# albertgassol1/vf-nerf

Measured on AMD Instinct MI355X. Metric: rays/sec (4096-ray chunk, 128 samples/ray) + PSNR vs ref, higher is better.
Workload: dtype f16x3+f32acc

## Files before the change

vf_nerf_amd/csrc/vfn_mlp16.hip:

```cpp
#include <string.h>
#include <utility>
#include "vfn_common.h"
#include "vfn_plan.h"

typedef _Float16 half8 __attribute__((ext_vector_type(8)));
typedef _Float16 half2v __attribute__((ext_vector_type(2)));
typedef float float2v __attribute__((ext_vector_type(2)));
typedef float f32x16 __attribute__((ext_vector_type(16)));
typedef float f32x4v __attribute__((ext_vector_type(4)));

constexpr float VFN16_WSCALE = 64.0f;
constexpr float VFN16_INV_WSCALE = 0.015625f;
constexpr float VFN16_XSCALE = 64.0f;
constexpr int VFN16_SAVE_AUX = 2;
constexpr int VFN16_HANDOVER_NUM = 8;
constexpr int VFN16_DMA_STEPS = 16;
constexpr int VFN16_EPI_PER_MFMA = 6;
constexpr int VFN16_EPI_PER_MFMA2 = 9;
#define VFN16_MAX_CHUNK_KB 39
#define VFN16_STATS_WORDS 64

struct Plan16 {
    int32_t n_hidden;
    int32_t feat_layer;
// ... 180 lines not shown
        }
    }
    {
        Pack16Entry& e = a.e[a.n_entries++];
        rc = fill(e, L - 1);
        if (rc != VFN_OK) return rc;
        e.off_kb = p.head_off_kb; e.n_chunks = 1; e.act16 = 16; e.aux16 = 0;
        e.row_off = 0; e.n_rows = 3; e.act_col_off = 0; e.act_valid = VFN_HIDDEN;
    }
    a.total_words = p.total_kb * 256u;
    a.out = (uint32_t*)packed16;
    a.stats = a.out + a.total_words;
    if (hipMemsetAsync(a.stats, 0, VFN16_STATS_WORDS * 4, (hipStream_t)stream) != hipSuccess) {
        vfn_set_error("vfn_pack16_weights: hipMemsetAsync failed");
        return VFN_ERR_LAUNCH;
    }
    hipLaunchKernelGGL(vfn_pack16_kernel, dim3(a.total_words / 256 + VFN16_STAT_WGS * a.n_entries), dim3(256), 0, (hipStream_t)stream, a);
    return vfn_check_launch("vfn_pack16_weights");
}

namespace {

enum : int { EPI_RELU = 0, EPI_TANH = 1, EPI_HEAD_TANH = 2, EPI_HEAD_SIGMOID = 3 };
enum : int { M16_FEAT = 1, M16_RENDER = 2, M16_TRAIN = 4, M16_BLKOUT = 8, M16_BLKIN = 16, M16_C2 = 32, M16_P1 = 64, M16_SF16 = 128,
             M16_VF_VEC = 0, M16_FUSED = M16_FEAT | M16_RENDER, M16_VF_BLK = M16_FEAT | M16_BLKOUT, M16_RN_BLK = M16_RENDER | M16_BLKIN,
             M16_VF_VEC_TRAIN = M16_TRAIN, M16_VF_FULL_TRAIN = M16_FEAT | M16_TRAIN, M16_FUSED_TRAIN = M16_FUSED | M16_TRAIN };

constexpr int VFN16_FDEPTH = 2;
#define VFN16_SLOT (VFN16_MAX_CHUNK_KB * 64)
#define VFN16_WAVES 4
#define VFN16_PTS 128

typedef __attribute__((address_space(3))) void lds_void;

constexpr int VF_ACT[9] = {0, 16, 16, 16, 14, 16, 16, 16, 16};
constexpr int VF_AUX[9] = {3, 0, 0, 0, 3, 0, 0, 0, 0};
constexpr int VF_TILES[9] = {8, 8, 8, 7, 8, 8, 8, 8, 8};
constexpr int RN_ACT[4] = {16, 16, 16, 16};
constexpr int RN_AUX[4] = {3, 0, 0, 0};
constexpr int RN_TILES[4] = {8, 8, 8, 8};
constexpr int HEAD_KB = 2 * 16 + 1;
constexpr int chunk_kb(int act, int aux) { return 2 * (act + aux) + 1; }
constexpr int vf_off_kb(int h) { int o = 0; for (int i = 0; i < h; ++i) o += VF_TILES[i] * chunk_kb(VF_ACT[i], VF_AUX[i]); return o; }
constexpr int rn_off_kb(int h) { int o = 0; for (int i = 0; i < h; ++i) o += RN_TILES[i] * chunk_kb(RN_ACT[i], RN_AUX[i]); return o; }

struct ChunkD { int net, off_kb, kb, aux; };
constexpr ChunkD chunk_of(int mode, int c) {
    if (!(mode & M16_BLKIN)) {
        const int vf_layers = (mode & M16_FEAT) ? 9 : 8;
        for (int h = 0; h < vf_layers; ++h) {
            if (c < VF_TILES[h]) return {0, vf_off_kb(h) + c * chunk_kb(VF_ACT[h], VF_AUX[h]), chunk_kb(VF_ACT[h], VF_AUX[h]), VF_AUX[h]};
            c -= VF_TILES[h];
        }
        if (c == 0) return {0, vf_off_kb(9), HEAD_KB, 0};
        c -= 1;
    }
    if (mode & M16_RENDER) {
        for (int h = 0; h < 4; ++h) {
            if (c < RN_TILES[h]) return {1, rn_off_kb(h) + c * chunk_kb(RN_ACT[h], RN_AUX[h]), chunk_kb(RN_ACT[h], RN_AUX[h]), RN_AUX[h]};
            c -= RN_TILES[h];
        }
        if (c == 0) return {1, rn_off_kb(4), HEAD_KB, 0};
    }
    return {0, 0, 0, 0};
}

constexpr int rn_first_chunk(int mode) { return (mode & M16_BLKIN) ? 0 : 72; }
constexpr bool chunk_two(int mode, int c) { return (mode & M16_C2) && !(mode & M16_BLKIN) && c >= 63 && c != 71; }
constexpr bool mode_one(int mode) { return (mode & M16_P1) != 0; }
constexpr int VFN16_P1_RING = 5;
#define VFN16_P1_SLOT_KB 20
constexpr int ring_of(int mode) { return mode_one(mode) ? VFN16_P1_RING : 3; }
constexpr int slot_u4(int mode) { return mode_one(mode) ? VFN16_P1_SLOT_KB * 64 : VFN16_MAX_CHUNK_KB * 64; }
constexpr int slot_base(int mode, int c) { return (c % ring_of(mode)) * slot_u4(mode); }
static_assert(VFN16_P1_RING * VFN16_P1_SLOT_KB <= 3 * VFN16_MAX_CHUNK_KB, "the single-product ring must fit into the split modes' ring");
constexpr int stores_of(int mode, int c) { return (c == 0 || ((mode & M16_RENDER) && c == rn_first_chunk(mode))) ? 0 : 4; }
constexpr int young_ops(int mode, int c) {
    const int ring = ring_of(mode);
    int n = 0;
    for (int k = (c - ring + 2 > 0 ? c - ring + 2 : 0); k < c; ++k) n += stores_of(mode, k);
    for (int j = 2; j <= ring - 2; ++j)
        if (c + j >= ring - 1 && chunk_of(mode, c + j).kb > 0) n += (((chunk_of(mode, c + j).kb - 1) / 2 + 1) / VFN16_WAVES);
    return n;
}

struct Mlp16Args {
    const uint4* vf_w;
    const uint4* rn_w;
    const float* points;
    const float* ray_dirs;
    float* out_vec;
    float* out_colors;
    long long n_points;
    int dirs_div;
    int vf_multires, rn_multires;
    uint32_t vf_bytes, rn_bytes;
    float* saved;
    float* save_aux_vf;
    float* save_aux_rn;
    uint32_t* save_masks;
    int save_f16;
    uint4* blk_out;
    const uint4* blk_in;
    const float* vec_in;
    const int* src;
    const int* out_index;
    long long ws_first, ws_points;
    uint32_t* status;
    const int* n_dev;
    unsigned long long* clock;
    long long clock_slots;
};

#define VFN16_CLAMP 60000.0f
constexpr int VFN16_CLAMP_BITS = 0x476a6000;
static_assert(__builtin_bit_cast(int, VFN16_CLAMP) == VFN16_CLAMP_BITS, "VFN16_CLAMP_BITS is VFN16_CLAMP as an integer");

struct X16 { half8 hi[16]; half8 lo[16]; };
struct A16 { half8 hi[3]; half8 lo[3]; };

struct Pipe16 {
    uint4* lds;
    __amdgpu_buffer_rsrc_t vf_w;
    __amdgpu_buffer_rsrc_t rn_w;
    float* saved;
    long long slot_floats;
    uint32_t slot_bytes;
    uint32_t save_voff;
    uint32_t save_voff16;
    uint32_t feat_voff;
    uint32_t st_tile, st_q;
    int save16;
    uint32_t* masks;
    uint32_t mask_bytes;
    uint32_t mask_voff;
    uint4* blk_out;
    uint32_t blk_bytes, blk_voff;
};

struct Carry16 {
    f32x16 pend;
    f32x16 bias;
    half8 fh0, fl0;
    uint32_t lm[4];
    unsigned long long sat;
};

template <int N, typename F, int... I>
__device__ __forceinline__ void static_for_impl(F&& f, std::integer_sequence<int, I...>) { (f(std::integral_constant<int, I>{}), ...); }
template <int N, typename F>
__device__ __forceinline__ void static_for(F&& f) { static_for_impl<N>(f, std::make_integer_sequence<int, N>{}); }

__device__ __forceinline__ void split2(float a, float b, _Float16& h0, _Float16& h1, _Float16& l0, _Float16& l1) {
    const float2v v = {a, b};
    const half2v hi = __builtin_convertvector(v, half2v);
    h0 = hi[0]; h1 = hi[1];
    const uint32_t hp = __builtin_bit_cast(uint32_t, hi);
    float r0, r1;
    asm("v_fma_mix_f32 %0, %1, -1.0, %2 op_sel_hi:[1,0,0]" : "=v"(r0) : "v"(hp), "v"(a));
    asm("v_fma_mix_f32 %0, %1, -1.0, %2 op_sel:[1,0,0] op_sel_hi:[1,0,0]" : "=v"(r1) : "v"(hp), "v"(b));
    const float2v r = {r0, r1};
    const half2v lo = __builtin_convertvector(r, half2v);
    l0 = lo[0]; l1 = lo[1];
}

__device__ __forceinline__ float tanh_exp(float v) { return 1.0f - 2.0f / (1.0f + expf(2.0f * v)); }
// ... 221 lines not shown
                else asm volatile("s_waitcnt vmcnt(0)" ::: "memory");
                __builtin_amdgcn_s_barrier();
            }
            if (st >= H && st < H + DST && ddma.kb > 0) {
#pragma unroll
                for (int i = (st - H) * PM / DST; i < (st - H + 1) * PM / DST; ++i) {
                    if (VFN16_WAVES * i + VFN16_WAVES <= DPIECES) dma_piece<ddma.net, ddma.off_kb, slot_base(MODE, C + RING - 1)>(p, piece_blk(wave + VFN16_WAVES * i), lane, P1 ? wave + VFN16_WAVES * i : -1);
                    else if (VFN16_WAVES * i < DPIECES) {
                        const int idx = min(wave + VFN16_WAVES * i, DPIECES - 1);
                        dma_piece<ddma.net, ddma.off_kb, slot_base(MODE, C + RING - 1)>(p, piece_blk(idx), lane, P1 ? idx : -1);
                    }
                }
            }
            if (TRAIN && MPARTS > 0 && st >= H && st < H + MPARTS && (ch > 0 || PEPI >= 0)) {
                static_for<MPARTS>([&](auto ip) {
                    constexpr int part = decltype(ip)::value;
                    if (st - H == part) {
                        if (ch > 0) collect_mask_part<(ch > 0 ? ch - 1 : 0), EPI, part, (MPARTS > 0 ? MPARTS : 1)>(cy, mbits);
                        else collect_mask_part<PKB / 2, (PEPI >= 0 ? PEPI : 0), part, (MPARTS > 0 ? MPARTS : 1)>(cy, mbits);
                    }
                });
            }
            if (TRAIN && st >= DEND && st < DEND + SSTEPS && (ch > 0 || PEPI >= 0)) {
                if (st == DEND) {
                    if constexpr (MPARTS > 0) {
                        if (ch == 0) store_mask<(PSLOT >= 0 ? PSLOT : 0)>(p, cy);
                    } else {
                        if (ch > 0) collect_mask<(ch > 0 ? ch - 1 : 0), EPI>(cy);
                        else { collect_mask<PKB / 2, (PEPI >= 0 ? PEPI : 0)>(cy); store_mask<(PSLOT >= 0 ? PSLOT : 0)>(p, cy); }
                    }
                }
#pragma unroll
                for (int q = (st - DEND) * 4 / SSTEPS; q < (st - DEND + 1) * 4 / SSTEPS; ++q) {
                    if (ch > 0) save_group<(SLOT >= 0 ? SLOT : 0), (ch > 0 ? ch - 1 : 0), (MODE & M16_SF16) != 0>(p, cy.pend, q);
                    else save_group<(PSLOT >= 0 ? PSLOT : 0), PKB / 2, (MODE & M16_SF16) != 0>(p, cy.pend, q);
                }
            }
            if (st == H && ((BLK && ch > 0) || (PBLK && ch == 0))) {
                if (ch > 0) store_blocks<(ch > 0 ? ch - 1 : 0)>(p, xout);
                else store_blocks<PKB / 2>(p, xpend);
            }
            if (st == NKB - 1 && dnext.kb > 0) prefetch_chunk<MODE, (dnext.kb > 0 ? C + 1 : C)>(cy, p, lane);
            __builtin_amdgcn_sched_barrier(0);
        }
        if (EPI == EPI_RELU || EPI == EPI_TANH) {
            cy.pend = acc;
        } else {
#pragma unroll
            for (int c = 0; c < 3; ++c) {
                const float v = acc[c] * VFN16_INV_WSCALE;
                head[c] = (EPI == EPI_HEAD_TANH) ? tanh_exp(v) : 1.0f / (1.0f + expf(-v));
            }
        }
    });
}

constexpr int ENC_RT = -1;
constexpr int VFN16_VF_MULTIRES = 6, VFN16_RN_MULTIRES = 4;
constexpr int enc_multires(int fixed, int run_time) { return fixed >= 0 ? fixed : run_time; }

__device__ __forceinline__ void lane_half_pair(float v, float& low, float& high) {
    const unsigned u = __builtin_bit_cast(unsigned, v);
    const auto r = __builtin_amdgcn_permlane32_swap(u, u, false, false);
    low = __builtin_bit_cast(float, (unsigned)r[0]); high = __builtin_bit_cast(float, (unsigned)r[1]);
}

__device__ __forceinline__ float enc_value(const float (&x)[3], const float (&sn)[18], const float (&cs)[18], int multires, int k) {
    if (k < 3) return x[k];
    const int idx = k - 3, oct = idx / 6, rem = idx - 6 * oct;
    if (oct >= multires) return 0.f;
    return rem < 3 ? sn[3 * oct + rem] : cs[3 * oct + rem - 3];
}

template <int NDEF, int NRAW, typename F>
__device__ __forceinline__ void build_aux(A16& aux, int g, F col, float& ain) {
    static_for<3>([&](auto is) {
        constexpr int s = decltype(is)::value;
        half8 hi, lo;
        static_for<4>([&](auto ij) {
            constexpr int j = 2 * decltype(ij)::value;
            if constexpr (16 * s + j >= NDEF) {
                hi[j] = (_Float16)0.f; hi[j + 1] = (_Float16)0.f; lo[j] = (_Float16)0.f; lo[j + 1] = (_Float16)0.f;
            } else {
                float v0, v1;
                if (g == 0) { v0 = col(16 * s + j); v1 = col(16 * s + j + 1); }
                else { v0 = col(16 * s + 8 + j); v1 = col(16 * s + 8 + j + 1); }
                v0 *= VFN16_XSCALE; v1 *= VFN16_XSCALE;
                v0 = fminf(fmaxf(v0, -VFN16_CLAMP), VFN16_CLAMP); v1 = fminf(fmaxf(v1, -VFN16_CLAMP), VFN16_CLAMP);
                if constexpr (16 * s + j < NRAW) ain = fmaxf(ain, fmaxf(fabsf(v0), fabsf(v1)));
                _Float16 h0, h1, l0, l1;
                split2(v0, v1, h0, h1, l0, l1);
                hi[j] = h0; hi[j + 1] = h1; lo[j] = l0; lo[j + 1] = l1;
            }
        });
        aux.hi[s] = hi; aux.lo[s] = lo;
    });
}

template <typename F>
__device__ __forceinline__ void save_aux(float* dst, long long m, int g, F col) {
#pragma unroll
    for (int s = 0; s < 3; ++s)
#pragma unroll
        for (int h = 0; h < 2; ++h) {
            const int c0 = 16 * s + 8 * g + 4 * h;
            if (c0 + 4 <= VFN_AUX_K) {
                f32x4v v;
                if (g == 0) { v = f32x4v{col(16 * s + 4 * h), col(16 * s + 4 * h + 1), col(16 * s + 4 * h + 2), col(16 * s + 4 * h + 3)}; }
                else { v = f32x4v{col(16 * s + 8 + 4 * h), col(16 * s + 8 + 4 * h + 1), col(16 * s + 8 + 4 * h + 2), col(16 * s + 8 + 4 * h + 3)}; }
                *reinterpret_cast<f32x4v*>(dst + m * VFN_AUX_K + c0) = v;
            }
        }
}

__device__ __forceinline__ void load_aux(A16& ax, const float* park) {
    const half8* pk = reinterpret_cast<const half8*>(park + 8);
#pragma unroll
    for (int q = 0; q < 3; ++q) { ax.hi[q] = pk[2 * q]; ax.lo[q] = pk[2 * q + 1]; }
}

template <int MR>
__device__ __forceinline__ void encode_sincos(const float (&x)[3], int multires_rt, int g, float (&sn)[18], float (&cs)[18]) {
    const int multires = enc_multires(MR, multires_rt);
#pragma unroll
    for (int j = 0; j < 3; ++j)
#pragma unroll
        for (int c = 0; c < 3; ++c) {
            if (MR >= 0 && 2 * j >= MR) {
                sn[6 * j + c] = 0.f; cs[6 * j + c] = 0.f; sn[6 * j + 3 + c] = 0.f; cs[6 * j + 3 + c] = 0.f;
                continue;
            }
            float s = 0.f, k = 0.f;
            if (2 * j < multires) {
                sincosf(x[c] * (g ? (float)(2 << (2 * j)) : (float)(1 << (2 * j))), &s, &k);
                if (g && 2 * j + 1 >= multires) { s = 0.f; k = 0.f; }
            }
            lane_half_pair(s, sn[6 * j + c], sn[6 * j + 3 + c]);
            lane_half_pair(k, cs[6 * j + c], cs[6 * j + 3 + c]);
        }
}

template <int MODE, int RNM>
__device__ __forceinline__ void render_aux(const Mlp16Args& a, A16& aux, const float (&xr)[3], const float (&dr)[3], const float (&nrm)[3],
                                           long long m, bool in, int g, float& ain) {
    const int rn_multires = enc_multires(RNM, a.rn_multires);
    float sn[18], cs[18];
    encode_sincos<RNM>(dr, rn_multires, g, sn, cs);
    const int ncol = 6 + 6 * rn_multires;
    auto rn_col = [&](int k) -> float {
        if (k < 3) return xr[k];
        if (k >= ncol) return k < ncol + 3 ? nrm[k - ncol] : 0.f;
        return enc_value(dr, sn, cs, rn_multires, k - 3);
    };
    build_aux<(RNM >= 0 ? 9 + 6 * RNM : 48), 6>(aux, g, rn_col, ain);
    if ((MODE & M16_TRAIN) && in) save_aux(a.save_aux_rn, m, g, rn_col);
}

template <int MODE>
__device__ __forceinline__ void render_tail(const Mlp16Args& a, const Pipe16& p, Carry16& cy, X16& xa, X16& xb, const A16& aux,
                                            const float (&nrm)[3], long long m, bool in, int wave, int lane) {
    constexpr int R = EPI_RELU, NONE = -1;
    constexpr int C0 = rn_first_chunk(MODE);
    float rgb[3] = {0.f, 0.f, 0.f};
    layer16<MODE, C0 + 0, 16, 3, 8, R, NONE, 0, 9, -1>(xb, aux, xa, xb, cy, rgb, p, wave, lane);
    layer16<MODE, C0 + 8, 16, 0, 8, R, R, 14, 10, 9>(xa, aux, xb, xa, cy, rgb, p, wave, lane);
    layer16<MODE, C0 + 16, 16, 0, 8, R, R, 14, 11, 10>(xb, aux, xa, xb, cy, rgb, p, wave, lane);
    layer16<MODE, C0 + 24, 16, 0, 8, R, R, 14, 12, 11>(xa, aux, xb, xa, cy, rgb, p, wave, lane);
    layer16<MODE, C0 + 32, 16, 0, 1, EPI_HEAD_SIGMOID, R, 14, -1, 12>(xb, aux, xa, xb, cy, rgb, p, wave, lane);
    const long long mo = m;
    if (in && (threadIdx.x & 32) == 0) {
        a.out_vec[mo * 3 + 0] = nrm[0]; a.out_vec[mo * 3 + 1] = nrm[1]; a.out_vec[mo * 3 + 2] = nrm[2];
        a.out_colors[mo * 3 + 0] = rgb[0]; a.out_colors[mo * 3 + 1] = rgb[1]; a.out_colors[mo * 3 + 2] = rgb[2];
    }
}

__device__ __forceinline__ void report_range(const Mlp16Args& a, unsigned long long sat, float ain) {
    if (a.status) {
        const unsigned bits = (sat != 0ull ? 1u : 0u) | (ain >= VFN16_CLAMP ? 2u : 0u);
        if (bits) atomicOr(a.status, bits);
    }
}

template <int MODE, int VFM, int RNM>
__device__ __forceinline__ void mlp16_body(const Mlp16Args& a) {
    __shared__ __attribute__((aligned(16))) uint4 s_ring[3 * VFN16_SLOT + 256 * 8];
    float* s_park = reinterpret_cast<float*>(s_ring + 3 * VFN16_SLOT) + threadIdx.x * 32;
    const int tid = threadIdx.x;
    const int lane = tid & 63;
    const int wave = __builtin_amdgcn_readfirstlane(tid >> 6);
    const int g = lane >> 5;
    unsigned long long ck_t0 = 0ull, ck_r0 = 0ull;
    if constexpr ((MODE & M16_RENDER) != 0 && (MODE & M16_BLKIN) == 0 && (MODE & M16_TRAIN) == 0) {
        if (a.clock) { ck_t0 = __builtin_amdgcn_s_memtime(); ck_r0 = __builtin_amdgcn_s_memrealtime(); }
    }
    const long long m = (long long)blockIdx.x * VFN16_PTS + wave * 32 + (lane & 31);
    long long n_live = a.n_points;
    if (a.n_dev) {
        const long long nd = (long long)*a.n_dev;
        n_live = nd < n_live ? nd : n_live;
        if ((long long)blockIdx.x * VFN16_PTS >= n_live) return;
    }
    const bool in = m < n_live;

    if constexpr ((MODE & M16_BLKIN) != 0) {
        const int dpos = in ? a.src[m] : -1;
        const bool live = dpos >= 0;
        float xr[3] = {0.f, 0.f, 0.f}, dr[3] = {0.f, 0.f, 0.f}, nrm[3] = {0.f, 0.f, 0.f};
        if (live) {
            const long long di = dpos / a.dirs_div;
#pragma unroll
            for (int c = 0; c < 3; ++c) { xr[c] = a.points[(long long)dpos * 3 + c]; dr[c] = a.ray_dirs[di * 3 + c]; nrm[c] = a.vec_in[m * 3 + c]; }
        }
        Pipe16 p;
        p.lds = s_ring;
        p.vf_w = __builtin_amdgcn_make_buffer_rsrc(const_cast<uint4*>(a.rn_w), 0, (int)a.rn_bytes, 0x00020000);
        p.rn_w = p.vf_w;
        p.saved = nullptr; p.slot_floats = 0; p.slot_bytes = 0; p.save_voff = 0; p.blk_out = nullptr; p.blk_bytes = 0; p.blk_voff = 0;
        p.masks = nullptr; p.mask_bytes = 0; p.mask_voff = 0; p.save16 = 0; p.save_voff16 = 0; p.feat_voff = 0; p.st_tile = 0; p.st_q = 0;
        dma_chunk<MODE, 0>(p, wave, lane);
        dma_chunk<MODE, 1>(p, wave, lane);
        X16 xa, xb;
        A16 aux;
        float ain_blk = 0.f;
        {
            typedef unsigned int u32x4 __attribute__((ext_vector_type(4)));
            const __amdgpu_buffer_rsrc_t rs_blk = __builtin_amdgcn_make_buffer_rsrc(
                const_cast<uint4*>(a.blk_in), 0, (int)(((a.n_points + 31) & ~31ll) * 1024), 0x00020000);
            const unsigned goff = in ? (unsigned)((m >> 5) * 32768 + lane * 16) : 0xfffffff0u;
            u32x4 q[32];
#pragma unroll
            for (int i = 0; i < 32; ++i) q[i] = __builtin_amdgcn_raw_buffer_load_b128(rs_blk, goff, i * 1024, 0);
            render_aux<MODE, RNM>(a, aux, xr, dr, nrm, -1, false, g, ain_blk);
#pragma unroll
            for (int t = 0; t < 8; ++t) {
                half8 h0 = __builtin_bit_cast(half8, q[4 * t + 0]), l0 = __builtin_bit_cast(half8, q[4 * t + 1]);
                half8 h1 = __builtin_bit_cast(half8, q[4 * t + 2]), l1 = __builtin_bit_cast(half8, q[4 * t + 3]);
                asm volatile("" : "+a"(h0)); asm volatile("" : "+a"(l0)); asm volatile("" : "+a"(h1)); asm volatile("" : "+a"(l1));
                xb.hi[2 * t] = h0; xb.lo[2 * t] = l0; xb.hi[2 * t + 1] = h1; xb.lo[2 * t + 1] = l1;
            }
        }
        asm volatile("s_waitcnt vmcnt(0)" ::: "memory");
        __builtin_amdgcn_s_barrier();
        Carry16 cy;
#pragma unroll
        for (int q = 0; q < 16; ++q) cy.pend[q] = 0.f;
        cy.lm[0] = 0; cy.lm[1] = 0; cy.lm[2] = 0; cy.lm[3] = 0; cy.sat = 0ull;
        prefetch_chunk<MODE, 0>(cy, p, lane);
        render_tail<MODE>(a, p, cy, xa, xb, aux, nrm, live ? (long long)dpos : -1, live, wave, lane);
        report_range(a, cy.sat, ain_blk);
    } else {
    float x[3] = {0.f, 0.f, 0.f};
    if (in) { x[0] = a.points[m * 3 + 0]; x[1] = a.points[m * 3 + 1]; x[2] = a.points[m * 3 + 2]; }
    float d[3] = {0.f, 0.f, 0.f};
    int out_row = -1;
    if ((MODE & M16_RENDER) && in) {
        const long long di = m / a.dirs_div;
        d[0] = a.ray_dirs[di * 3 + 0]; d[1] = a.ray_dirs[di * 3 + 1]; d[2] = a.ray_dirs[di * 3 + 2];
        if (a.out_index) out_row = a.out_index[m];
    }
    asm volatile("s_waitcnt vmcnt(0)" ::: "memory");
    if (MODE & M16_RENDER) {
        s_park[0] = x[0]; s_park[1] = x[1]; s_park[2] = x[2];
        s_park[4] = d[0]; s_park[5] = d[1]; s_park[6] = d[2];
    }

    Pipe16 p;
    p.lds = s_ring;
    p.vf_w = __builtin_amdgcn_make_buffer_rsrc(const_cast<uint4*>(a.vf_w), 0, (int)a.vf_bytes, 0x00020000);
    p.rn_w = __builtin_amdgcn_make_buffer_rsrc(const_cast<uint4*>((MODE & M16_RENDER) ? a.rn_w : a.vf_w), 0,
                                               (int)((MODE & M16_RENDER) ? a.rn_bytes : a.vf_bytes), 0x00020000);
    const bool frag = (a.save_f16 & 2) != 0;
    const long long mw = m + a.ws_first;
    p.slot_floats = frag ? ((a.ws_points + 31) >> 5) * 8192 : a.ws_points * 256;
    p.saved = a.saved + a.ws_first * 256;
    {
        const long long left = p.slot_floats * 4 - a.ws_first * 1024;
        p.slot_bytes = (uint32_t)(left < 0x7fffffffll ? left : 0x7fffffffll);
    }
    p.save_voff = !in ? (frag ? 0xc0000000u : 0xfffffff0u) : (frag ? (uint32_t)((m >> 5) * 32768 + lane * 16) : (uint32_t)(m * 1024 + g * 16));
    p.save_voff16 = !in ? (frag ? 0xc0000000u : 0xfffffff0u) : (frag ? (uint32_t)((m >> 5) * 32768 + lane * 8) : (uint32_t)(m * 1024 + g * 8));
    p.feat_voff = in ? (uint32_t)(m * 1024 + g * 16) : 0xfffffff0u;
    p.st_tile = frag ? 4096u : 128u; p.st_q = frag ? 1024u : 32u;
    p.masks = a.save_masks; p.mask_bytes = (uint32_t)(a.ws_points * 32); p.mask_voff = in ? (uint32_t)((2 * mw + g) * 16) : 0xfffffff0u;
    p.save16 = a.save_f16 & 1;
    p.blk_out = a.blk_out; p.blk_bytes = (uint32_t)(((a.n_points + 31) & ~31ll) * 1024);
    p.blk_voff = (uint32_t)((m >> 5) * 32768 + lane * 16);
    dma_chunk<MODE, 0>(p, wave, lane);
    dma_chunk<MODE, 1>(p, wave, lane);
    if constexpr (mode_one(MODE)) static_for<VFN16_P1_RING - 3>([&](auto ic) { dma_chunk<MODE, 2 + decltype(ic)::value>(p, wave, lane); });

    const int vf_multires = enc_multires(VFM, a.vf_multires);
    A16 aux;
    float ain = 0.f;
    {
        float sn[18], cs[18];
        encode_sincos<VFM>(x, vf_multires, g, sn, cs);
        build_aux<(VFM >= 0 ? 3 + 6 * VFM : 48), 3>(aux, g, [&](int k) { return enc_value(x, sn, cs, vf_multires, k); }, ain);
        if ((MODE & M16_TRAIN) && in) save_aux(a.save_aux_vf, mw, g, [&](int k) { return enc_value(x, sn, cs, vf_multires, k); });
        half8* pk = reinterpret_cast<half8*>(s_park + 8);
#pragma unroll
        for (int q = 0; q < 3; ++q) { pk[2 * q] = aux.hi[q]; pk[2 * q + 1] = aux.lo[q]; }
    }
    asm volatile("s_waitcnt vmcnt(0)" ::: "memory");
    __builtin_amdgcn_s_barrier();
    Carry16 cy;
#pragma unroll
    for (int q = 0; q < 16; ++q) cy.pend[q] = 0.f;
    cy.lm[0] = 0; cy.lm[1] = 0; cy.lm[2] = 0; cy.lm[3] = 0; cy.sat = 0ull;
    prefetch_chunk<MODE, 0>(cy, p, lane);

    X16 xa, xb;
    float vec[3] = {0.f, 0.f, 0.f};
    constexpr int R = EPI_RELU, T = EPI_TANH, NONE = -1;
    layer16<MODE, 0, 0, 3, 8, R, NONE, 0, 0, -1>(xa, aux, xb, xb, cy, vec, p, wave, lane);
    layer16<MODE, 8, 16, 0, 8, R, R, 14, 1, 0>(xb, aux, xa, xb, cy, vec, p, wave, lane);
    layer16<MODE, 16, 16, 0, 8, R, R, 14, 2, 1>(xa, aux, xb, xa, cy, vec, p, wave, lane);
    layer16<MODE, 24, 16, 0, 7, R, R, 14, 3, 2>(xb, aux, xa, xb, cy, vec, p, wave, lane);
    { A16 ax; load_aux(ax, s_park); layer16<MODE, 31, 14, 3, 8, R, R, 12, 4, 3>(xa, ax, xb, xa, cy, vec, p, wave, lane); }
    layer16<MODE, 39, 16, 0, 8, R, R, 14, 5, 4>(xb, aux, xa, xb, cy, vec, p, wave, lane);
    layer16<MODE, 47, 16, 0, 8, R, R, 14, 6, 5>(xa, aux, xb, xa, cy, vec, p, wave, lane);
    layer16<MODE, 55, 16, 0, 8, R, R, 14, 7, 6>(xb, aux, xa, xb, cy, vec, p, wave, lane);
    if constexpr (!(MODE & M16_FEAT)) {
        layer16<MODE, 63, 16, 0, 1, EPI_HEAD_TANH, R, 14, -1, 7>(xa, aux, xb, xa, cy, vec, p, wave, lane);
        if (in && g == 0) { a.out_vec[m * 3 + 0] = vec[0]; a.out_vec[m * 3 + 1] = vec[1]; a.out_vec[m * 3 + 2] = vec[2]; }
        report_range(a, cy.sat, ain);
    } else {
    constexpr bool BO = (MODE & M16_BLKOUT) != 0;
    layer16<MODE, 63, 16, 0, 8, T, R, 14, 8, 7, BO, false>(xa, aux, xb, xa, cy, vec, p, wave, lane);
    layer16<MODE, 71, 16, 0, 1, EPI_HEAD_TANH, T, 14, -1, 8, false, BO>(xa, aux, xb, xb, cy, vec, p, wave, lane);
    if constexpr (!(MODE & M16_RENDER)) {
        if (in && g == 0) { a.out_vec[m * 3 + 0] = vec[0]; a.out_vec[m * 3 + 1] = vec[1]; a.out_vec[m * 3 + 2] = vec[2]; }
        report_range(a, cy.sat, ain);
    } else {
    float nrm[3];
#pragma unroll
    for (int c = 0; c < 3; ++c) { float upper; lane_half_pair(vec[c], nrm[c], upper); }
    const float xr[3] = {s_park[0], s_park[1], s_park[2]};
    const float dr[3] = {s_park[4], s_park[5], s_park[6]};
    A16 raux;
    render_aux<MODE, RNM>(a, raux, xr, dr, nrm, (MODE & M16_TRAIN) ? mw : m, in, g, ain);
    render_tail<MODE>(a, p, cy, xa, xb, raux, nrm, a.out_index ? (long long)out_row : m, a.out_index ? out_row >= 0 : in, wave, lane);
    report_range(a, cy.sat, ain);
    if constexpr ((MODE & M16_TRAIN) == 0) {
        if (a.clock && threadIdx.x == 0 && (long long)blockIdx.x < a.clock_slots) {
            const unsigned long long t1 = __builtin_amdgcn_s_memtime(), r1 = __builtin_amdgcn_s_memrealtime();
            a.clock[2 * blockIdx.x] = t1 - ck_t0; a.clock[2 * blockIdx.x + 1] = r1 - ck_r0;
        }
    }
    }
    }
    }
}

constexpr bool enc_fixed(int mode) { return (mode & M16_TRAIN) == 0; }

template <int MODE>
__global__ __launch_bounds__(256, 1) void vfn_mlp16_kernel(const Mlp16Args a) {
    mlp16_body<MODE, (enc_fixed(MODE) ? VFN16_VF_MULTIRES : ENC_RT), (enc_fixed(MODE) ? VFN16_RN_MULTIRES : ENC_RT)>(a);
}

template <int MODE>
__global__ __launch_bounds__(256, 1) void vfn_mlp16_anyenc_kernel(const Mlp16Args a) {
    mlp16_body<MODE, ENC_RT, ENC_RT>(a);
}

template <int MODE>
void launch16(const Mlp16Args& a, long long blocks, void* stream) {
    static_assert(enc_fixed(MODE), "training modes have one kernel");
    const bool vf_ok = (MODE & M16_BLKIN) != 0 || a.vf_multires == VFN16_VF_MULTIRES;
    const bool rn_ok = (MODE & M16_RENDER) == 0 || a.rn_multires == VFN16_RN_MULTIRES;
    if (vf_ok && rn_ok) hipLaunchKernelGGL(vfn_mlp16_kernel<MODE>, dim3((unsigned)blocks), dim3(256), 0, (hipStream_t)stream, a);
    else hipLaunchKernelGGL(vfn_mlp16_anyenc_kernel<MODE>, dim3((unsigned)blocks), dim3(256), 0, (hipStream_t)stream, a);
}

int check_vf16(const Plan16& vf, const char* what) {
    bool ok = vf.feat_layer == 1 && vf.n_hidden == 9 && (int)vf.head_off_kb == vf_off_kb(9);
    for (int h = 0; ok && h < 9; ++h)
        ok = vf.act16[h] == VF_ACT[h] && vf.aux16[h] == VF_AUX[h] && vf.n_tiles[h] == VF_TILES[h] && (int)vf.off_kb[h] == vf_off_kb(h);
    if (!ok) { vfn_set_error("%s: the f16x3 kernels are specialised for the shipped vector-field network shape", what); return VFN_ERR_UNSUPPORTED; }
    return VFN_OK;
}
int check_rn16(const Plan16& rn, const char* what) {
    bool ok = rn.n_hidden == 4 && (int)rn.head_off_kb == rn_off_kb(4);
    for (int h = 0; ok && h < 4; ++h)
        ok = rn.act16[h] == RN_ACT[h] && rn.aux16[h] == RN_AUX[h] && rn.n_tiles[h] == RN_TILES[h] && (int)rn.off_kb[h] == rn_off_kb(h);
    if (!ok) { vfn_set_error("%s: the f16x3 kernels are specialised for the shipped rendering network shape", what); return VFN_ERR_UNSUPPORTED; }
    return VFN_OK;
}

}

static int check_kind16(int net_kind, const Plan16& p, const char* what) {
    return net_kind == VFN_NET_VF ? check_vf16(p, what) : check_rn16(p, what);
}

static thread_local uint32_t* t_status_word = nullptr;

uint32_t* vfn_internal_f16x3_status() { return t_status_word; }

extern "C" int vfn_f16x3_set_status(uint32_t* status_word) {
    t_status_word = status_word;
    return VFN_OK;
}

static thread_local unsigned long long* t_clock_probe = nullptr;
static thread_local long long t_clock_slots = 0;

extern "C" int vfn_f16x3_set_clock_probe(uint64_t* stamps, int64_t slots) {
    VFN_REQUIRE(slots >= 0 && (stamps || slots == 0), "vfn_f16x3_set_clock_probe: %lld slots without a buffer", (long long)slots);
    t_clock_probe = reinterpret_cast<unsigned long long*>(stamps);
    t_clock_slots = stamps ? slots : 0;
    return VFN_OK;
}

VfnReportScope::VfnReportScope(uint32_t* status_word, uint64_t* clock_stamps, int64_t clock_slots)
    : old_status(t_status_word), old_clock(t_clock_probe), old_slots(t_clock_slots) {
    if (status_word) t_status_word = status_word;
    if (clock_stamps && clock_slots > 0) { t_clock_probe = reinterpret_cast<unsigned long long*>(clock_stamps); t_clock_slots = clock_slots; }
}
VfnReportScope::~VfnReportScope() { t_status_word = old_status; t_clock_probe = old_clock; t_clock_slots = old_slots; }

extern "C" int vfn_vf_mlp16_fwd(const vfn_net_geom* geom, const void* packed16, const float* points, int64_t n_points,
                                 float* out_vec, void* stream) {
    Mlp16Args a = {};
// ... 223 lines not shown
```

Measured before the change: 2.073 million.

## Overlap point/direction loads with weight DMA and share per-ray direction encoding

In inference render mode, point and ray-direction loads are issued as untracked dwordx3 loads and waited on only after the first weight-chunk DMAs, using a partial vmcnt, so global latency overlaps the prologue. The rendering network's direction encoding is computed once per ray when a wave holds a single ray: lanes compute different sincos terms and broadcast them with readlane, falling back to the per-lane path otherwise. The direction/position part of the render aux is built early and parked in extra LDS, and only the normal columns are patched in later. This costs more LDS, readlane traffic and register pressure, and relies on the hand-computed vmcnt count being correct.

```diff
diff --git a/vf_nerf_amd/csrc/vfn_mlp16.hip b/vf_nerf_amd/csrc/vfn_mlp16.hip
--- a/vf_nerf_amd/csrc/vfn_mlp16.hip
+++ b/vf_nerf_amd/csrc/vfn_mlp16.hip
@@ -286,6 +286,26 @@
     for (int j = 2; j <= ring - 2; ++j)
         if (c + j >= ring - 1 && chunk_of(mode, c + j).kb > 0) n += (((chunk_of(mode, c + j).kb - 1) / 2 + 1) / VFN16_WAVES);
     return n;
+}
+
+typedef float f32x3v __attribute__((ext_vector_type(3)));
+__device__ __forceinline__ f32x3v load3_untracked(const float* p) {
+    f32x3v v;
+    asm volatile("global_load_dwordx3 %0, %1, off" : "=v"(v) : "v"(p) : "memory");
+    return v;
+}
+
+constexpr int prologue_pieces(int mode) {
+    int least = 1 << 30;
+    for (int w = 0; w < VFN16_WAVES; ++w) {
+        int n = 0;
+        for (int c = 0; c < ring_of(mode) - 1; ++c) {
+            const int pieces = mode_one(mode) ? (chunk_of(mode, c).kb - 1) / 2 + 1 : chunk_of(mode, c).kb;
+            for (int i = 0; w + VFN16_WAVES * i < pieces; ++i) ++n;
+        }
+        least = n < least ? n : least;
+    }
+    return least;
 }
 
 struct Mlp16Args {
@@ -673,9 +693,8 @@
             if constexpr (16 * s + j >= NDEF) {
                 hi[j] = (_Float16)0.f; hi[j + 1] = (_Float16)0.f; lo[j] = (_Float16)0.f; lo[j + 1] = (_Float16)0.f;
             } else {
-                float v0, v1;
-                if (g == 0) { v0 = col(16 * s + j); v1 = col(16 * s + j + 1); }
-                else { v0 = col(16 * s + 8 + j); v1 = col(16 * s + 8 + j + 1); }
+                const float a0 = col(16 * s + j), a1 = col(16 * s + j + 1), b0 = col(16 * s + 8 + j), b1 = col(16 * s + 8 + j + 1);
+                float v0 = g == 0 ? a0 : b0, v1 = g == 0 ? a1 : b1;
                 v0 *= VFN16_XSCALE; v1 *= VFN16_XSCALE;
                 v0 = fminf(fmaxf(v0, -VFN16_CLAMP), VFN16_CLAMP); v1 = fminf(fmaxf(v1, -VFN16_CLAMP), VFN16_CLAMP);
                 if constexpr (16 * s + j < NRAW) ain = fmaxf(ain, fmaxf(fabsf(v0), fabsf(v1)));
@@ -713,14 +732,11 @@
 template <int MR>
 __device__ __forceinline__ void encode_sincos(const float (&x)[3], int multires_rt, int g, float (&sn)[18], float (&cs)[18]) {
     const int multires = enc_multires(MR, multires_rt);
-#pragma unroll
-    for (int j = 0; j < 3; ++j)
-#pragma unroll
-        for (int c = 0; c < 3; ++c) {
-            if (MR >= 0 && 2 * j >= MR) {
-                sn[6 * j + c] = 0.f; cs[6 * j + c] = 0.f; sn[6 * j + 3 + c] = 0.f; cs[6 * j + 3 + c] = 0.f;
-                continue;
-            }
+    static_for<9>([&](auto ijc) {
+        constexpr int j = decltype(ijc)::value / 3, c = decltype(ijc)::value % 3;
+        if constexpr (MR >= 0 && 2 * j >= MR) {
+            sn[6 * j + c] = 0.f; cs[6 * j + c] = 0.f; sn[6 * j + 3 + c] = 0.f; cs[6 * j + 3 + c] = 0.f;
+        } else {
             float s = 0.f, k = 0.f;
             if (2 * j < multires) {
                 sincosf(x[c] * (g ? (float)(2 << (2 * j)) : (float)(1 << (2 * j))), &s, &k);
@@ -729,14 +745,46 @@
             lane_half_pair(s, sn[6 * j + c], sn[6 * j + 3 + c]);
             lane_half_pair(k, cs[6 * j + c], cs[6 * j + 3 + c]);
         }
-}
-
-template <int MODE, int RNM>
+    });
+}
+
+template <int RNM>
+__device__ __forceinline__ void encode_direction(const float (&dr)[3], int multires_rt, long long di, bool in, int lane, int g,
+                                                 float (&sn)[18], float (&cs)[18]) {
+    constexpr int NL = RNM >= 0 ? 3 * RNM : 18;
+    const unsigned long long live = __builtin_amdgcn_ballot_w64(in);
+    const int first = live ? __builtin_ctzll(live) : 0;
+    const int di_lo = (int)di, di_hi = (int)(di >> 32);
+    const int first_lo = __builtin_amdgcn_readlane(di_lo, first), first_hi = __builtin_amdgcn_readlane(di_hi, first);
+    const bool one_ray = __builtin_amdgcn_ballot_w64(in && (di_lo != first_lo || di_hi != first_hi)) == 0ull;
+    float s = 0.f, k = 0.f;
+    if (one_ray) {
+        const float du0 = __builtin_bit_cast(float, __builtin_amdgcn_readlane(__builtin_bit_cast(int, dr[0]), first));
+        const float du1 = __builtin_bit_cast(float, __builtin_amdgcn_readlane(__builtin_bit_cast(int, dr[1]), first));
+        const float du2 = __builtin_bit_cast(float, __builtin_amdgcn_readlane(__builtin_bit_cast(int, dr[2]), first));
+        const int l = lane < NL ? lane : 0;
+        const int o = l / 3, c = l - 3 * o;
+        sincosf((c == 0 ? du0 : (c == 1 ? du1 : du2)) * __builtin_bit_cast(float, (127 + o) << 23), &s, &k);
+    } else {
+        encode_sincos<RNM>(dr, multires_rt, g, sn, cs);
+    }
+    if (one_ray) {
+        static_for<NL>([&](auto ii) {
+            constexpr int i = decltype(ii)::value;
+            const float si = __builtin_bit_cast(float, __builtin_amdgcn_readlane(__builtin_bit_cast(int, s), i));
+            const float ki = __builtin_bit_cast(float, __builtin_amdgcn_readlane(__builtin_bit_cast(int, k), i));
+            sn[i] = in ? si : 0.f; cs[i] = in ? ki : 1.f;
+        });
+    }
+}
+
+template <int MODE, int RNM, bool SHARE = false>
 __device__ __forceinline__ void render_aux(const Mlp16Args& a, A16& aux, const float (&xr)[3], const float (&dr)[3], const float (&nrm)[3],
-                                           long long m, bool in, int g, float& ain) {
+                                           long long m, bool in, int g, float& ain, long long di = -1, int lane = 0) {
     const int rn_multires = enc_multires(RNM, a.rn_multires);
     float sn[18], cs[18];
-    encode_sincos<RNM>(dr, rn_multires, g, sn, cs);
+    if constexpr (SHARE) encode_direction<RNM>(dr, rn_multires, di, in, lane, g, sn, cs);
+    else encode_sincos<RNM>(dr, rn_multires, g, sn, cs);
     const int ncol = 6 + 6 * rn_multires;
     auto rn_col = [&](int k) -> float {
         if (k < 3) return xr[k];
@@ -745,6 +793,57 @@
     };
     build_aux<(RNM >= 0 ? 9 + 6 * RNM : 48), 6>(aux, g, rn_col, ain);
     if ((MODE & M16_TRAIN) && in) save_aux(a.save_aux_rn, m, g, rn_col);
+}
+
+constexpr int VFN16_HEAD_BLOCKS = 2;
+template <int RNM>
+__device__ __forceinline__ void render_aux_head(half8* park_a, half8* park_b, const float (&xr)[3], const float (&dr)[3], long long di,
+                                                bool in, int lane, int g, float& ain) {
+    static_assert(RNM >= 0 && 6 + 6 * RNM <= 16 * VFN16_HEAD_BLOCKS, "the columns in front of the normal fill two K-blocks at most");
+    float sn[18], cs[18];
+    encode_direction<RNM>(dr, RNM, di, in, lane, g, sn, cs);
+    constexpr int ncol = 6 + 6 * RNM;
+    auto rn_col = [&](int k) -> float {
+        if (k < 3) return xr[k];
+        if (k >= ncol) return 0.f;
+        return enc_value(dr, sn, cs, RNM, k - 3);
+    };
+    A16 aux;
+    build_aux<9 + 6 * RNM, 6>(aux, g, rn_col, ain);
+    park_a[0] = aux.hi[0]; park_a[1] = aux.lo[0]; park_b[0] = aux.hi[1]; park_b[1] = aux.lo[1];
+}
+
+template <int RNM>
+__device__ __forceinline__ void render_aux_normal(A16& aux, const half8* park_a, const half8* park_b, const float (&nrm)[3], int g) {
+    typedef unsigned int u32x4 __attribute__((ext_vector_type(4)));
+    constexpr int ncol = 6 + 6 * RNM;
+    aux.hi[0] = park_a[0]; aux.lo[0] = park_a[1]; aux.hi[1] = park_b[0]; aux.lo[1] = park_b[1];
+#pragma unroll
+    for (int j = 0; j < 8; ++j) { aux.hi[2][j] = (_Float16)0.f; aux.lo[2][j] = (_Float16)0.f; }
+    const float pair[2][2] = {{nrm[0], nrm[1]}, {nrm[2], 0.f}};
+    uint32_t hp[2], lp[2];
+#pragma unroll
+    for (int q = 0; q < 2; ++q) {
+        float v0 = pair[q][0] * VFN16_XSCALE, v1 = pair[q][1] * VFN16_XSCALE;
+        v0 = fminf(fmaxf(v0, -VFN16_CLAMP), VFN16_CLAMP); v1 = fminf(fmaxf(v1, -VFN16_CLAMP), VFN16_CLAMP);
+        _Float16 h0, h1, l0, l1;
+        split2(v0, v1, h0, h1, l0, l1);
+        const half2v h = {h0, h1}, l = {l0, l1};
+        hp[q] = __builtin_bit_cast(uint32_t, h); lp[q] = __builtin_bit_cast(uint32_t, l);
+    }
+    static_for<3>([&](auto is) {
+        constexpr int s = decltype(is)::value;
+        u32x4 hi = __builtin_bit_cast(u32x4, aux.hi[s]), lo = __builtin_bit_cast(u32x4, aux.lo[s]);
+        static_for<4>([&](auto ij) {
+            constexpr int jj = decltype(ij)::value;
+            if constexpr (16 * s + 2 * jj < 9 + 6 * RNM) {
+                const int k = 16 * s + 8 * g + 2 * jj;
+                hi[jj] = k == ncol ? hp[0] : (k == ncol + 2 ? hp[1] : hi[jj]);
+                lo[jj] = k == ncol ? lp[0] : (k == ncol + 2 ? lp[1] : lo[jj]);
+            }
+        });
+        aux.hi[s] = __builtin_bit_cast(half8, hi); aux.lo[s] = __builtin_bit_cast(half8, lo);
+    });
 }
 
 template <int MODE>
@@ -774,8 +873,9 @@
 
 template <int MODE, int VFM, int RNM>
 __device__ __forceinline__ void mlp16_body(const Mlp16Args& a) {
-    __shared__ __attribute__((aligned(16))) uint4 s_ring[3 * VFN16_SLOT + 256 * 8];
+    __shared__ __attribute__((aligned(16))) uint4 s_ring[3 * VFN16_SLOT + 256 * 8 + 256 * 2];
     float* s_park = reinterpret_cast<float*>(s_ring + 3 * VFN16_SLOT) + threadIdx.x * 32;
+    [[maybe_unused]] half8* s_park_b = reinterpret_cast<half8*>(s_ring + 3 * VFN16_SLOT + 256 * 8) + threadIdx.x * 2;
     const int tid = threadIdx.x;
     const int lane = tid & 63;
     const int wave = __builtin_amdgcn_readfirstlane(tid >> 6);
@@ -840,19 +940,34 @@
         render_tail<MODE>(a, p, cy, xa, xb, aux, nrm, live ? (long long)dpos : -1, live, wave, lane);
         report_range(a, cy.sat, ain_blk);
     } else {
+    constexpr bool INFER = (MODE & M16_RENDER) != 0 && (MODE & M16_TRAIN) == 0;
+    constexpr bool EARLY = INFER && RNM >= 0;
     float x[3] = {0.f, 0.f, 0.f};
-    if (in) { x[0] = a.points[m * 3 + 0]; x[1] = a.points[m * 3 + 1]; x[2] = a.points[m * 3 + 2]; }
     float d[3] = {0.f, 0.f, 0.f};
     int out_row = -1;
+    [[maybe_unused]] long long dir_row = -1;
+    [[maybe_unused]] f32x3v xq = {0.f, 0.f, 0.f}, dq = {0.f, 0.f, 0.f};
+    if constexpr (INFER) {
+        if (in) {
+            dir_row = m / a.dirs_div;
+            xq = load3_untracked(a.points + m * 3);
+            dq = load3_untracked(a.ray_dirs + dir_row * 3);
+            if (a.out_index) out_row = a.out_index[m];
+        }
+    } else {
+    if (in) { x[0] = a.points[m * 3 + 0]; x[1] = a.points[m * 3 + 1]; x[2] = a.points[m * 3 + 2]; }
     if ((MODE & M16_RENDER) && in) {
         const long long di = m / a.dirs_div;
         d[0] = a.ray_dirs[di * 3 + 0]; d[1] = a.ray_dirs[di * 3 + 1]; d[2] = a.ray_dirs[di * 3 + 2];
         if (a.out_index) out_row = a.out_index[m];
     }
+    }
+    if constexpr (!INFER) {
     asm volatile("s_waitcnt vmcnt(0)" ::: "memory");
     if (MODE & M16_RENDER) {
         s_park[0] = x[0]; s_park[1] = x[1]; s_park[2] = x[2];
         s_park[4] = d[0]; s_park[5] = d[1]; s_park[6] = d[2];
+    }
     }
 
     Pipe16 p;
@@ -879,10 +994,20 @@
     dma_chunk<MODE, 0>(p, wave, lane);
     dma_chunk<MODE, 1>(p, wave, lane);
     if constexpr (mode_one(MODE)) static_for<VFN16_P1_RING - 3>([&](auto ic) { dma_chunk<MODE, 2 + decltype(ic)::value>(p, wave, lane); });
+    if constexpr (INFER) {
+        static_assert(prologue_pieces(MODE) < 64, "vmcnt is a 6-bit field");
+        asm volatile("s_waitcnt vmcnt(%2)" : "+v"(xq), "+v"(dq) : "n"(prologue_pieces(MODE)) : "memory");
+        x[0] = xq[0]; x[1] = xq[1]; x[2] = xq[2]; d[0] = dq[0]; d[1] = dq[1]; d[2] = dq[2];
+        if constexpr (!EARLY) {
+            s_park[0] = x[0]; s_park[1] = x[1]; s_park[2] = x[2]; s_park[3] = __builtin_bit_cast(float, (int)dir_row);
+            s_park[4] = d[0]; s_park[5] = d[1]; s_park[6] = d[2]; s_park[7] = __builtin_bit_cast(float, (int)(dir_row >> 32));
+        }
+    }
 
     const int vf_multires = enc_multires(VFM, a.vf_multires);
     A16 aux;
     float ain = 0.f;
+    if constexpr (EARLY) render_aux_head<RNM>(reinterpret_cast<half8*>(s_park), s_park_b, x, d, dir_row, in, lane, g, ain);
     {
         float sn[18], cs[18];
         encode_sincos<VFM>(x, vf_multires, g, sn, cs);
@@ -926,11 +1051,18 @@
     float nrm[3];
 #pragma unroll
     for (int c = 0; c < 3; ++c) { float upper; lane_half_pair(vec[c], nrm[c], upper); }
-    const float xr[3] = {s_park[0], s_park[1], s_park[2]};
-    const float dr[3] = {s_park[4], s_park[5], s_park[6]};
     A16 raux;
-    render_aux<MODE, RNM>(a, raux, xr, dr, nrm, (MODE & M16_TRAIN) ? mw : m, in, g, ain);
-    render_tail<MODE>(a, p, cy, xa, xb, raux, nrm, a.out_index ? (long long)out_row : m, a.out_index ? out_row >= 0 : in, wave, lane);
+    if constexpr (EARLY) {
+        render_aux_normal<RNM>(raux, reinterpret_cast<const half8*>(s_park), s_park_b, nrm, g);
+    } else {
+        const float xr[3] = {s_park[0], s_park[1], s_park[2]};
+        const float dr[3] = {s_park[4], s_park[5], s_park[6]};
+        const long long di = INFER ? (long long)(((unsigned long long)__builtin_bit_cast(unsigned, s_park[7]) << 32) | __builtin_bit_cast(unsigned, s_park[3])) : -1ll;
+        render_aux<MODE, RNM, INFER>(a, raux, xr, dr, nrm, (MODE & M16_TRAIN) ? mw : m, in, g, ain, di, lane);
+    }
+    int wave_rn = wave;
+    if constexpr (EARLY) asm volatile("" : "+s"(wave_rn));
+    render_tail<MODE>(a, p, cy, xa, xb, raux, nrm, a.out_index ? (long long)out_row : m, a.out_index ? out_row >= 0 : in, wave_rn, lane);
     report_range(a, cy.sat, ain);
     if constexpr ((MODE & M16_TRAIN) == 0) {
         if (a.clock && threadIdx.x == 0 && (long long)blockIdx.x < a.clock_slots) {
```

Result: no change. 2.076 million (median of 4 runs) (+0.1%).
